# tudelft/event_flow

Hardware: AMD Instinct MI355X
Metric: event-windows/sec (train step, 128x128x15k ev) (higher is better)
Workload: dtype f32

## Files before the change

event_flow_amd/_lib.py:

```python

import ctypes
import os

import torch

_HERE = os.path.dirname(os.path.abspath(__file__))
LIB_PATH = os.environ.get("EVF_LIB") or os.path.join(_HERE, "libevflow_hip.so")

P = ctypes.c_void_p
I = ctypes.c_int
F = ctypes.c_float
L = ctypes.c_int64

SIGNATURES = {
    "evf_version": [],
    "evf_device_count": [],
    "evf_events_to_image": [P, P, P, I, I, I, I, P, P],
    "evf_encode_events": [P, I, I, I, I, I, I, P, P, P, P, P],
    "evf_encode_window": [P, I, I, I, I, I, I, I, I, P, P, P],
    "evf_iwe_splat": [P, P, P, P, P, P, I, I, I, I, I, F, F, F, I, I, P, P],
    "evf_get_interpolation": [P, P, I, I, I, I, F, F, I, P, P, P],
    "evf_interpolate": [P, P, P, I, I, I, I, I, P, P],
    "evf_cm_smooth_blocks": [I, I, I, I],
    "evf_norm_nonzero": [P, ctypes.c_int64, P, P, P],
# ... 62 lines not shown
    "evf_head_dgrad_win_fits": [I, I, I, I, I, I, I, I, I],
    "evf_head_dgrad_win_select": [I, I],
    "evf_head_bwd_dgrad_win": [P, P, P, P, P, P, P, P, P, I, I, I, I, I, I, F, P, P, P, P, I, P],
    "evf_sum_rows": [P, I, I, I, P, P],
    "evf_add_segments": [P, P, P, P, I, I, P],
    "evf_pack_conv_weights_b3_multi": [P, P, P, I, P],
    "evf_reduce_slabs_multi": [P, P, I, I, I, P],
    "evf_lif_bwd_wgrad": [P, P, P, P, P, P, P, P, P, I, I, I, I, I, F, P, P, P, P, P, P, P, I, P],
    "evf_lif_bwd_wgrad2": [P, P, P, P, P, P, P, P, P, P, I, I, I, I, I, F, P, P, P, P, P, P, P, I, P],
    "evf_lif_bwd_wgrad_top": [P, P, P, P, P, P, P, P, P, P, P, P, P, I, I, I, I, I, F, P, P, P, P, P, P, I, P],
    "evf_debug_poison_lds": [ctypes.c_uint32, P],
    "evf_memset": [P, I, ctypes.c_size_t, P],
    "evf_plif_bwd_wgrad2": [P, P, P, P, P, P, P, P, P, P, I, I, I, I, I, F, P, P, P, P, P, P, P, I, P, P, P, P, P, P, P, P, P, P],
    "evf_conv_dgrad_b3_multi": [I, P, P, P, P, P, I, I, I, P],
    "evf_conv_dgrad_b3_multi_fits": [I, I, I],
    "evf_lif_bwd_wgrad_window": [I, P, P, P, P, P, P, P, P, P, P, P, P, P, P, P, I, I, I, F, P, P, P, P, I, P],
    "evf_plif_bwd_wgrad_window_top": [I, P, P, P, P, P, P, P, P, P, P, P, P, P, P, P, P, P, P, P, I, I, I, F, P, P, P, P, P, P, P, I, P],
    "evf_plif_bwd_wgrad_window": [I, P, P, P, P, P, P, P, P, P, P, P, P, P, P, I, I, I, F, P, P, P, P, P, P, P, I, P],
    "evf_plif_bwd_wgrad_top": [P, P, P, P, P, P, P, P, P, P, P, P, P, I, I, I, I, I, F, P, P, P, P, P, P, I,
                               P, P, P, P, P, P, P, P, P, P],
    "evf_pack_conv_weight_b3t": [P, I, I, P, P],
    "evf_conv_dgrad_b3": [P, P, P, I, I, I, I, P, P, P],
    "evf_conv_dgrad_b3_f32": [P, P, P, I, I, I, I, P, P, P],
    "evf_conv_dgrad_select": [I],
    "evf_dgrad_diag_select": [I],
    "evf_bwd_diag_select": [I],
    "evf_bwd_leak_defer": [],
    "evf_fwd_diag_select": [I],
    "evf_conv_dgrad_b3_f32_pair": [P, P, P, I, P, P, I, I, I, P, P, P],
    "evf_conv_dgrad_b3_pair": [P, P, P, I, P, P, I, I, I, P, P, P],
# ... 295 lines not shown
```

event_flow_amd/csrc/evf_bwd_fused.hip:

```cpp
#include <stdio.h>

#include "evf_common.h"
#include "evf_split.h"
#include <stdlib.h>
#include <mutex>

typedef float f32x16 __attribute__((ext_vector_type(16)));
typedef __bf16 bf16x8 __attribute__((ext_vector_type(8)));

#define C32 32
#define FB_CW 64
#define FB_UNITS 8
#define FB_UNITS_MAX 64
#define FB_THREADS 512
#define FB_NW (FB_CW / 32 + 2)
#define FB_R0 32768

#define FB_LD_SKIP 16
#define FB_LD_COLLECT 32
#define FB_LD_MIN_LEAK (-11.0f)

__device__ __forceinline__ int fb_row(int r, int lane) { return (r & 3) + 8 * (r >> 2) + 4 * (lane >> 5); }
__device__ __forceinline__ float fb_sigmoid(float x) { return 1.0f / (1.0f + expf(-x)); }
__device__ __forceinline__ uint32_t fb_bf16(float f) {
// ... 226 lines not shown
        dlam = vp[c] * (1.0f - z) - cur;
      } else {
        gp[c] = gv * lam[c];
        cur = (vo[c] - vp[c] * lam[c] + z * th[c]) * inv_oml[c];
        dlam = vp[c] - cur;
        if (ok) st[c] -= gv * z;
      }
      if (ok) {
        sl[c] += gv * dlam;
        st[c] -= gsp;
      }
    }
    if (ok) {
#ifdef FB_NT_STORES
      if (g_cur) g_cur[pix0 * 8 + tid] = make_float4(gc[0], gc[1], gc[2], gc[3]);
      evf_store_nt(g_v_prev + pix0 * 8 + tid, make_float4(gp[0], gp[1], gp[2], gp[3]));
#else
      if (g_cur) g_cur[pix0 * 8 + tid] = make_float4(gc[0], gc[1], gc[2], gc[3]);
      g_v_prev[pix0 * 8 + tid] = make_float4(gp[0], gp[1], gp[2], gp[3]);
#endif
    }
    uint32_t tp[3][2];
    const int base = ((p >> 3) * C32) * 8 + (p & 7);
#pragma unroll
    for (int e = 0; e < 2; ++e) {
      evf_split3_pair(ok ? gc[2 * e] : 0.f, ok ? gc[2 * e + 1] : 0.f, tp[0][e], tp[1][e], tp[2][e]);
#pragma unroll
      for (int t3 = 0; t3 < 3; ++t3) {
        const int o = t3 * FB_CW * C32 + base + (4 * cg + 2 * e) * 8;
        sb[o] = (unsigned short)tp[t3][e];
        sb[o + 8] = (unsigned short)(tp[t3][e] >> 16);
      }
    }
    if (ok && g_split) {
// ... 503 lines not shown
          if (LD && ld_collect) sl[c] += (vo[c] * inv_oml[c]) * (gvo[c] * inv_lam[c]);
          st[c] -= gsp;
        }
        }
      }
      const long eo = pix0 * 8 + ETHR * h + et;
      if (WIN) {
        gvc = make_float4(gp[0], gp[1], gp[2], gp[3]);
        voc = vp4;
        if (ok) {
          if (w_gcur) w_gcur[eo] = make_float4(gc[0], gc[1], gc[2], gc[3]);
          if (ks == T - 1 && g_v_prev) g_v_prev[eo] = gvc;
        }
      } else if (ok) {
        if (g_cur) g_cur[eo] = make_float4(gc[0], gc[1], gc[2], gc[3]);
        g_v_prev[eo] = make_float4(gp[0], gp[1], gp[2], gp[3]);
      }
      if (PLIF) {
        const float4 gk4 = WIN ? (ks > 0 ? gkc : z4) : (has_gk ? sp.gk : z4), pp4 = (WIN ? w_pp : has_pp) ? sp.pp : z4;
        const float gk[4] = {gk4.x, gk4.y, gk4.z, gk4.w}, pp[4] = {pp4.x, pp4.y, pp4.z, pp4.w};
        const float Pv = sp.P;
        float gq[4], gPp = 0.f, gzx[4];
#pragma unroll
        for (int c = 0; c < 4; ++c) {
          const float po = pov[c];
          const float gx = xl ? gsv[c] : gc[c];
          const float g = gk[c] - apt[c] * gx;
          gq[c] = g * lpt[c];
          if constexpr (SOFT) gq[c] -= gzs[c] * apt[c];
          gzx[c] = g * (1.0f - lpt[c]);
          gPp += gzx[c];
// ... 903 lines not shown
  evf_bwd_defer_tab[c].active = false;
  evf_ctx_drop(c);
  return rc;
}

static int fb_launch(const float* g_z_out, const float* g_z_out2, const FbTop* topp, const float* g_v_out, const float* v_out, const float* v_prev,
                     const uint32_t* z_prev, const uint32_t* xT, const uint32_t* zT_prev, const float* leak,
                     const float* thresh, int B, int H, int W, int hard_reset, int surrogate, float act_width,
                     float* g_cur, void* g_split, float* g_v_prev, float* g_leak, float* g_thresh, float* slab_ff,
                     float* slab_rec, int accumulate, void* stream, const FbPlif* plp_ = nullptr) {
  if (plp_ && !((hard_reset != 0 || plp_->xl != 0) && surrogate == EVF_ARCTAN)) return EVF_ENOTSUP;
  FbPlif pl_arg = plp_ ? *plp_ : FbPlif{};
  pl_arg.soft = (plp_ && hard_reset == 0) ? 1 : 0;
  const FbPlif* plp = plp_ ? &pl_arg : nullptr;
  if (plp && plp->xl == 2 && topp) return EVF_ENOTSUP;
  if (!v_out || !xT || !leak || !thresh || (!g_cur && !g_split) || !g_v_prev || !g_leak || !g_thresh || !slab_ff || B <= 0 || H <= 0 ||
      W <= 0 || ((zT_prev != nullptr) != (slab_rec != nullptr)) || (topp && (g_z_out || zT_prev)) || (topp && g_z_out2))
    return EVF_EINVAL;
  const int row_ld = accumulate >> 8;
  const int ldf = (fb_leak_defer_env() && !plp) ? (accumulate & (FB_LD_SKIP | FB_LD_COLLECT)) : 0;
  accumulate = (accumulate & 1) | ldf;
  const long nunits = fb_units(B, H, W);
  const int nchunk = (W + FB_CW - 1) / FB_CW;
  const int nrows_all = fb_rows(nunits);
  dim3 grid(fb_blocks_per_cell(nunits, 1)), block(FB_THREADS);
  hipStream_t st = EVF_STREAM(stream);
  const FbTop top = topp ? *topp : FbTop{nullptr, nullptr, nullptr, nullptr, nullptr, nullptr};
  static bool attr[12] = {false};
  const bool fast = (hard_reset != 0 || plp != nullptr) && surrogate == EVF_ARCTAN;
  const int bctx = evf_ctx_find(stream);
  const EvfBwdDefer evf_bwd_defer = bctx >= 0 ? evf_bwd_defer_tab[bctx] : EvfBwdDefer{false, 0, false};
// ... 251 lines not shown
```

event_flow_amd/csrc/evf_common.h:

```cpp
#pragma once
#include <hip/hip_runtime.h>
#include <stdint.h>

#include "../../include/evflow.h"

#define EVF_STREAM(s) ((hipStream_t)(s))

static inline int evf_status() {
  hipError_t e = hipGetLastError();
  return e == hipSuccess ? EVF_OK : -(1000 + (int)e);
}
static inline int evf_hip(hipError_t e) { return e == hipSuccess ? EVF_OK : -(1000 + (int)e); }

#define EVF_KSZ_OK(k) ((k) == 1 || (k) == 3 || (k) == 5 || (k) == 7)

static inline int evf_cdiv(long a, long b) { return (int)((a + b - 1) / b); }

template <auto KERNEL>
static inline void evf_dynamic_lds_once(size_t bytes) {
  static const hipError_t once = hipFuncSetAttribute((const void*)KERNEL, hipFuncAttributeMaxDynamicSharedMemorySize, (int)bytes);
  (void)once;
}

static __global__ void k_evf_fill(uint32_t* __restrict__ dst, uint32_t word, size_t nwords, unsigned char* __restrict__ tail, int ntail,
// ... 132 lines not shown
      s += (raw ? in : (dy == 1 && dx == 1)) ? v : 0.f;
    }
  return raw ? (s / 9.0f) / 32.0f : s;
}

int evf_dgrad_ws_launch(const float* g_cur, const void* wT_b3, float* g_x, int accumulate, int B, int H, int W, const float* g_P,
                        const uint32_t* x_bits, const void* wT2_b3, float* g_x2, int max_blocks, void* stream);

#define EVF_DG_MAX_PROD 16
struct EvfDgProd {
  const void* g;
  const void* wt;
  float* gx;
  const float* gP;
  const uint32_t* xb;
};
struct EvfDgProds {
  EvfDgProd p[EVF_DG_MAX_PROD];
};
int evf_dgrad_diag_ws_launch(const EvfDgProds& P, int nprod, int B, int H, int W, void* stream);
int evf_dgrad_diag_dma_launch(const EvfDgProds& P, int nprod, int B, int H, int W, void* stream);
bool evf_dgrad_diag_fits(int split, int B, int H, int W);

#define EVF_HDW_MAX_P 16
struct EvfHdwArgs {
  const void* g[EVF_HDW_MAX_P];
  const float* v_prev[EVF_HDW_MAX_P];
  const uint32_t* z_prev[EVF_HDW_MAX_P];
  const float* x_in[EVF_HDW_MAX_P];
  const void* wt;
// ... 37 lines not shown
```

event_flow_amd/csrc/evf_dgrad_b3.hip:

```cpp
#include "evf_common.h"
#include "evf_dgrad_mma.h"
#include "evf_split.h"
#include <stdlib.h>

typedef float f32x16 __attribute__((ext_vector_type(16)));
typedef __bf16 bf16x8 __attribute__((ext_vector_type(8)));

#define C32 32
#define DG_ROWS 8
#define NFRAG 54

__device__ __forceinline__ int dg_row(int r, int lane) { return (r & 3) + 8 * (r >> 2) + 4 * (lane >> 5); }
__device__ __forceinline__ uint32_t dg_bf16(float f) {
  const uint32_t u = __float_as_uint(f);
  return (u + 0x7FFFu + ((u >> 16) & 1u)) >> 16;
}

__global__ void k_pack_conv_weight_b3t(const float* __restrict__ w, uint4* __restrict__ dst) {
  const int idx = blockIdx.x * blockDim.x + threadIdx.x;
  if (idx >= 18 * 64) return;
  const int lane = idx & 63, tm = idx >> 6, m = tm & 1, tau = tm >> 1;
  const int j = lane & 31, kg = lane >> 5;
  uint32_t t[3][8];
  for (int e = 0; e < 8; ++e) {
// ... 211 lines not shown
                                                                    const float* __restrict__ gPb,
                                                                    const uint32_t* __restrict__ xbits,
                                                                    const uint4* __restrict__ wt2,
                                                                    float* __restrict__ gx2) {
  dg_body<F32IN, ACC, PLIF, PAIR>(blockIdx.z, gridDim.z, gs, plane_stride, wt, gx, accumulate, B, H, W, gPb, xbits, wt2, gx2);
}

#define DG_MAX_JOBS 8
struct DgJob {
  const uint4* gs;
  const uint4* wt;
  float* gx;
  const uint4* wt2;
  float* gx2;
  int split;
};
struct DgJobs {
  DgJob j[DG_MAX_JOBS];
};
__global__ __launch_bounds__(DG_ROWS * 64) void k_dgrad_diag(DgJobs jobs, int B, int H, int W, int zb) {
  const int jb = blockIdx.z / zb, zz = blockIdx.z - jb * zb;
  const DgJob& J = jobs.j[jb];
  if (J.wt2)
    dg_body<true, false, false, true>(zz, zb, J.gs, 0, J.wt, J.gx, 0, B, H, W, nullptr, nullptr, J.wt2, J.gx2);
  else
    dg_body<true, false, false, false>(zz, zb, J.gs, 0, J.wt, J.gx, 0, B, H, W, nullptr, nullptr, nullptr, nullptr);
}

struct DgDefer {
  int B, H, W, split;
// ... 31 lines not shown
int evf_dg_defer_pending(int ctx, int d) { return dg_tab[ctx].n[d]; }
int evf_dg_defer_launch(int ctx, int d, void* stream) {
  DgDefer& dg_defer = dg_tab[ctx];
  const int n = dg_defer.n[d];
  if (!n) return EVF_OK;
  static const bool env_ws = []() {
    const char* e = getenv("EVF_DGRAD_DIAG");
    return !(e && e[0] == 'l');
  }();
  if (dg_defer.split || (dg_diag_select < 0 ? env_ws : dg_diag_select == 1)) {
    EvfDgProds P;
    int np = 0;
    for (int k = 0; k < n; ++k) {
      const DgJob& J = dg_defer.job[d][k];
      P.p[np++] = EvfDgProd{J.gs, J.wt, J.gx};
      if (J.wt2) P.p[np++] = EvfDgProd{J.gs, J.wt2, J.gx2};
    }
    for (int k = np; k < EVF_DG_MAX_PROD; ++k) P.p[k] = P.p[0];
    evf_prof_mark(2, 0, stream);
    const int rc = dg_defer.split ? evf_dgrad_diag_dma_launch(P, np, dg_defer.B, dg_defer.H, dg_defer.W, stream)
                                  : evf_dgrad_diag_ws_launch(P, np, dg_defer.B, dg_defer.H, dg_defer.W, stream);
    evf_prof_mark(2, 1, stream);
    dg_defer.n[d] = 0;
    return rc;
  }
  const size_t lds = dg_lds_bytes();
  static bool attr_set = false;
  if (!attr_set) {
    (void)hipFuncSetAttribute((const void*)k_dgrad_diag, hipFuncAttributeMaxDynamicSharedMemorySize, (int)lds);
    attr_set = true;
  }
// ... 11 lines not shown
static int dg_select = -1;
extern "C" int evf_conv_dgrad_select(int which) {
  if (which < -1 || which > 1) return EVF_EINVAL;
  dg_select = which;
  return EVF_OK;
}

static int dg_launch(const void* g, int f32in, const void* wT_b3, float* g_x, int accumulate, int B, int H, int W,
                     const float* g_P, const uint32_t* x_bits, const void* wT2_b3, float* g_x2, void* stream) {
  if (!g || !wT_b3 || !g_x || B <= 0 || H <= 0 || W <= 0 || ((g_P != nullptr) != (x_bits != nullptr)) ||
      ((wT2_b3 != nullptr) != (g_x2 != nullptr)))
    return EVF_EINVAL;
  const int bctx = evf_ctx_find(stream);
  const EvfBwdDefer evf_bwd_defer = bctx >= 0 ? evf_bwd_defer_tab[bctx] : EvfBwdDefer{false, 0, false};
  DgDefer& dg_defer = dg_tab[bctx < 0 ? 0 : bctx];
  if (evf_bwd_defer.active) {
    const bool any = evf_dg_defer_count(bctx) != 0;
    const int split = f32in ? 0 : 1;
    const bool same = !any || (dg_defer.B == B && dg_defer.H == H && dg_defer.W == W && dg_defer.split == split);
    if (!accumulate && !g_P && same && dg_defer.n[evf_bwd_defer.slot] < DG_MAX_JOBS && evf_dgrad_diag_fits(split, B, H, W)) {
      dg_defer.B = B, dg_defer.H = H, dg_defer.W = W, dg_defer.split = split;
      dg_defer.job[evf_bwd_defer.slot][dg_defer.n[evf_bwd_defer.slot]++] =
          DgJob{(const uint4*)g, (const uint4*)wT_b3, g_x, (const uint4*)wT2_b3, g_x2, split};
      return EVF_OK;
    }
    const int rc = evf_bwd_defer_flush_now(bctx, stream);
    if (rc) return rc;
  }
  if (f32in) {
    int mode = dg_select;
    if (mode < 0) {
      static const int env_mode = []() {
        const char* e = getenv("EVF_DGRAD");
        return !e ? -1 : (e[0] == 'l' ? 0 : (e[0] == 'w' ? 1 : -1));
      }();
      mode = env_mode;
    }
    if (mode < 0) mode = ((long)B * evf_cdiv(H, 4) * evf_cdiv(W, 32) >= 6L * 256) ? 1 : 0;
    if (mode == 1)
      return evf_dgrad_ws_launch((const float*)g, wT_b3, g_x, accumulate, B, H, W, g_P, x_bits, wT2_b3, g_x2, 0, stream);
// ... 72 lines not shown
```

event_flow_amd/csrc/evf_dgrad_diag.hip:

```cpp
#include "evf_common.h"
#include "evf_dgrad_mma.h"
#include "evf_split.h"
#include <stdlib.h>
#include <type_traits>

typedef float f32x16 __attribute__((ext_vector_type(16)));
typedef __attribute__((address_space(3))) void wd_lds_void;
typedef __attribute__((address_space(1))) const void wd_glb_void;

#define C32 32
#define WD_ROWS 4
#define WD_HW 34
#define WD_HP ((WD_ROWS + 2) * WD_HW)
#define WD_NFRAG 54
#define WD_PLANE (WD_HP * 4)
#define WD_BUF (3 * WD_PLANE)
#define WD_ITEMS (WD_HP * 4)
#define WD_NIT ((WD_ITEMS + 255) / 256)
#define WD_SP 36
#define WD_LDS ((size_t)(WD_NFRAG * 64 + 2 * WD_BUF) * sizeof(uint4) + (size_t)WD_ROWS * 32 * WD_SP * 4)

#ifndef WD_PF
#define WD_PF 2
#endif
// ... 177 lines not shown
      __syncthreads();
    }
  }
  WD_STAMP();
}

#define WM_UPP 13
#define WM_PLANE (WM_UPP * 64)
#define WM_BUF (3 * WM_PLANE)
#define WM_NU (3 * WM_UPP)
#define WM_NJ ((WM_NU + 3) / 4)
#define WM_LDS ((size_t)(WD_NFRAG * 64 + 2 * WM_BUF) * sizeof(uint4) + (size_t)4 * 32 * WD_SP * 4)
#ifndef WM_STAGE
#define WM_STAGE 0
#endif
#ifndef WM_PIPE
#define WM_PIPE 1
#endif

__device__ uint4 wm_zero_page[16];

#ifdef WD_STAMPS
__device__ unsigned long long wm_stamps[16 * 4 * 128];
extern "C" int evf_debug_wm_stamps(void* dst) { return evf_hip(hipMemcpyFromSymbol(dst, HIP_SYMBOL(wm_stamps), sizeof(wm_stamps))); }
#define WM_STAMP()                                                                              \
  do {                                                                                          \
    if (blockIdx.x < 16 && lane == 0 && (wv & 3) == 0 && nst < 128)                             \
      wm_stamps[(blockIdx.x * 4 + (wv >> 2)) * 128 + nst++] = __builtin_readcyclecounter();     \
  } while (0)
#else
#define WM_STAMP() do {} while (0)
#endif

struct WmTile {
  int prod, b, y0, x0;
  const char* g;
  float* gx;
  const float* gP;
  const uint32_t* xb;
};

template <bool FULL, bool PLIFT = false>
__global__ __launch_bounds__(512) void k_dgrad_diag_dma(EvfDgProds P, unsigned plane_bytes, int H, int W, int ntx, int nty,
                                                        unsigned ntiles, unsigned total) {
  extern __shared__ __attribute__((aligned(16))) char smem_raw[];
  uint4* s_w = (uint4*)smem_raw;
  uint4* s_a = s_w + WD_NFRAG * 64;
  float* s_stage = (float*)(s_a + 2 * WM_BUF);
  const int tid = threadIdx.x, lane = tid & 63, wv = tid >> 6;
  const int i = lane & 31, kg = lane >> 5;
  int nst = 0;
  (void)nst;
  WM_STAMP();
  const unsigned lo = (unsigned)(((unsigned long long)blockIdx.x * total) / gridDim.x);
  const unsigned hi = (unsigned)(((unsigned long long)(blockIdx.x + 1) * total) / gridDim.x);
  const int nitem = (int)(hi - lo);
  if (nitem <= 0) return;
// ... 8 lines not shown
  auto item_of = [&](int k, WmTile& t) {
    const unsigned id = lo + (unsigned)min(k, nitem - 1);
    unsigned pr, tl, r, tx, b, ty;
    divmod(id, ntiles, rnt, pr, tl);
#ifdef WM_PROBE_COLMAJOR
    divmod(tl, (unsigned)nty, rnty, r, ty);
    divmod(r, (unsigned)ntx, rntx, b, tx);
#else
    divmod(tl, (unsigned)ntx, rntx, r, tx);
    divmod(r, (unsigned)nty, rnty, b, ty);
#endif
    t.prod = __builtin_amdgcn_readfirstlane((int)pr), t.x0 = __builtin_amdgcn_readfirstlane((int)tx * 32);
    t.b = __builtin_amdgcn_readfirstlane((int)b), t.y0 = __builtin_amdgcn_readfirstlane((int)ty * WD_ROWS);
    t.g = (const char*)P.p[t.prod].g, t.gx = P.p[t.prod].gx;
    if (PLIFT) t.gP = P.p[t.prod].gP, t.xb = P.p[t.prod].xb;
  };
  auto load_weights4 = [&](const uint4* src) {
    for (int u = wv - 4; u < WD_NFRAG; u += 4)
      __builtin_amdgcn_global_load_lds((wd_glb_void*)(src + u * 64 + lane), (wd_lds_void*)(s_w + u * 64), 16, 0, 0);
  };
  int p_hr[WM_NJ], p_hc[WM_NJ], p_lds[WM_NJ];
  unsigned p_off[WM_NJ];
#pragma unroll
  for (int j = 0; j < WM_NJ; ++j) {
    const int q = min((wv & 3) + 4 * j, WM_NU - 1), pl = q / WM_UPP, u = q - pl * WM_UPP;
    const int p = 16 * u + (lane >> 2), pc = min(p, WD_HP - 1);
    p_hr[j] = pc / WD_HW, p_hc[j] = pc - p_hr[j] * WD_HW;
    p_off[j] = (unsigned)pl * plane_bytes + (unsigned)(((lane & 3) ^ ((p >> 2) & 3)) * 16);
    p_lds[j] = __builtin_amdgcn_readfirstlane(pl * WM_PLANE + u * 64);
  }
// ... 26 lines not shown
  };
  float4 ev[4];
  auto epi_read = [&](int r) {
    const int p = 8 * r + (lane >> 3), c4 = (lane & 7) * 4;
    ev[r] = *(const float4*)(st + p * WD_SP + c4);
  };
  float gpv[9];
  uint32_t xbv = 0u;
  auto plif_load = [&](int r, const WmTile& t) {
    if (PLIFT && t.gP) {
      const int p = 8 * r + (lane >> 3);
      const int y = min(t.y0 + wv, H - 1), x = min(t.x0 + p, W - 1);
      evf_plif_gp_load(t.gP, 1, t.b, y, x, H, W, gpv);
      xbv = t.xb[((long)t.b * H + y) * W + x];
    }
  };
  auto epi_store = [&](int r, const WmTile& t) {
    const int y = t.y0 + wv;
    const int p = 8 * r + (lane >> 3), c4 = (lane & 7) * 4;
    float* dst = t.gx + ((unsigned)((t.b * H + y) * W + t.x0 + p) * (unsigned)C32 + (unsigned)c4);
    if (PLIFT && t.gP) {
      const float pv = evf_plif_gp_sum(1, min(y, H - 1), min(t.x0 + p, W - 1), H, W, gpv);
      const uint32_t xq = xbv >> c4;
      ev[r].x += (xq & 1u) ? pv : 0.f, ev[r].y += (xq & 2u) ? pv : 0.f, ev[r].z += (xq & 4u) ? pv : 0.f, ev[r].w += (xq & 8u) ? pv : 0.f;
    }
    if (FULL || (y < H && t.x0 + p < W)) evf_store_nt(dst, ev[r]);
  };
  WmTile cur, nxt, prv;
  int wprod;
  const bool loader = wv >= 4;
// ... 49 lines not shown
#endif
      WM_STAMP();
      __syncthreads();
      if (k + 1 < nitem && nxt.prod != wprod) {
        wprod = nxt.prod;
        load_weights4((const uint4*)P.p[wprod].wt);
        asm volatile("s_waitcnt vmcnt(0)" ::: "memory");
        __syncthreads();
      }
    }
  } else {
    f32x16 acc_prev = {0};
    auto run_item = [&](int k, auto epi_tag) {
      constexpr bool EPI = decltype(epi_tag)::value;
      WM_STAMP();
      auto side = [&](int slot) {
        if (slot == 70) item_of(k + 1, nxt);
        if (EPI) {
          if (slot == 1) epi_write(acc_prev);
#pragma unroll
          for (int r = 0; r < 4; ++r) {
            if (slot == 13 + r) epi_read(r);
            if (PLIFT && slot == 32 + 12 * r) plif_load(r, prv);
            if (slot == 40 + 12 * r) epi_store(r, prv);
          }
        }
      };
      const f32x16 acc = dg_matrix_phase3<WD_DPPX != 0>(s_w, s_a + (k & 1) * WM_BUF, WM_PLANE, wv * WD_HW + i, lane, side);
      WM_STAMP();
      if (!WM_PIPE) {
        epi_write(acc);
        __builtin_amdgcn_wave_barrier();
#pragma unroll
        for (int r = 0; r < 4; ++r) epi_read(r);
#pragma unroll
        for (int r = 0; r < 4; ++r) {
          plif_load(r, cur);
          epi_store(r, cur);
        }
        __builtin_amdgcn_wave_barrier();
      }
      acc_prev = acc;
      prv = cur;
      WM_STAMP();
      __syncthreads();
      if (k + 1 < nitem && nxt.prod != wprod) {
        wprod = nxt.prod;
        __syncthreads();
      }
      cur = nxt;
    };
    WM_STAMP();
    __syncthreads();
    prv = cur;
    run_item(0, std::false_type{});
    for (int k = 1; k < nitem; ++k) run_item(k, std::integral_constant<bool, WM_PIPE != 0>{});
    if (WM_PIPE) {
      epi_write(acc_prev);
      __builtin_amdgcn_wave_barrier();
#pragma unroll
      for (int r = 0; r < 4; ++r) epi_read(r);
#pragma unroll
      for (int r = 0; r < 4; ++r) {
        plif_load(r, prv);
        epi_store(r, prv);
      }
    }
  }
  WM_STAMP();
}

extern int evf_dgrad_ring_select;
#define WR_ROWS 12
#define WR_PITCH 36
#define WR_UPP 27
#define WR_PLANE (WR_UPP * 64)
// ... 238 lines not shown
  if (!attr) {
    (void)hipFuncSetAttribute((const void*)k_dgrad_diag_dma<true>, hipFuncAttributeMaxDynamicSharedMemorySize, (int)WM_LDS);
    (void)hipFuncSetAttribute((const void*)k_dgrad_diag_dma<false>, hipFuncAttributeMaxDynamicSharedMemorySize, (int)WM_LDS);
    attr = true;
  }
  const int nblk = (int)(total < ncu ? total : ncu);
  bool plift = false;
  for (int k = 0; k < nprod; ++k) {
    plift = plift || P.p[k].gP != nullptr;
    if (P.p[k].gP && !P.p[k].xb) return EVF_EINVAL;
  }
  static const bool ring_env = []() {
    const char* e = getenv("EVF_DGRAD_RING");
    return e && e[0] == '1';
  }();
  const bool ring = !plift && (evf_dgrad_ring_select < 0 ? ring_env : evf_dgrad_ring_select == 1);
  if (ring) {
    static bool rattr = false;
    if (!rattr) {
      (void)hipFuncSetAttribute((const void*)k_dgrad_diag_ring<true>, hipFuncAttributeMaxDynamicSharedMemorySize, (int)WR_LDS);
      (void)hipFuncSetAttribute((const void*)k_dgrad_diag_ring<false>, hipFuncAttributeMaxDynamicSharedMemorySize, (int)WR_LDS);
      rattr = true;
    }
    if (H % WD_ROWS == 0 && W % 32 == 0)
      hipLaunchKernelGGL(k_dgrad_diag_ring<true>, dim3(nblk), dim3(512), WR_LDS, EVF_STREAM(stream), P, (unsigned)plane_bytes, H, W,
                         ntx, nty, (unsigned)ntiles, (unsigned)total);
    else
      hipLaunchKernelGGL(k_dgrad_diag_ring<false>, dim3(nblk), dim3(512), WR_LDS, EVF_STREAM(stream), P, (unsigned)plane_bytes, H, W,
                         ntx, nty, (unsigned)ntiles, (unsigned)total);
    return evf_status();
// ... 15 lines not shown
  }
  if (H % WD_ROWS == 0 && W % 32 == 0)
    hipLaunchKernelGGL(k_dgrad_diag_dma<true>, dim3(nblk), dim3(512), WM_LDS, EVF_STREAM(stream), P, (unsigned)plane_bytes, H, W, ntx,
                       nty, (unsigned)ntiles, (unsigned)total);
  else
    hipLaunchKernelGGL(k_dgrad_diag_dma<false>, dim3(nblk), dim3(512), WM_LDS, EVF_STREAM(stream), P, (unsigned)plane_bytes, H, W, ntx,
                       nty, (unsigned)ntiles, (unsigned)total);
  return evf_status();
}

int evf_dgrad_diag_ws_launch(const EvfDgProds& P, int nprod, int B, int H, int W, void* stream) {
  if (nprod <= 0 || nprod > EVF_DG_MAX_PROD || B <= 0 || H <= 0 || W <= 0) return EVF_EINVAL;
  const int ntx = evf_cdiv(W, 32), nty = evf_cdiv(H, WD_ROWS);
  const long ntiles = (long)ntx * nty * B, total = ntiles * nprod;
  if (total >= (1L << 22)) return EVF_EINVAL;
  static int ncu = 0;
  if (!ncu) {
    int dev = 0;
    hipDeviceProp_t pr;
    if (hipGetDevice(&dev) == hipSuccess && hipGetDeviceProperties(&pr, dev) == hipSuccess) ncu = pr.multiProcessorCount;
    if (ncu <= 0) ncu = 256;
  }
  static bool attr = false;
  if (!attr) {
    (void)hipFuncSetAttribute((const void*)k_dgrad_diag_ws, hipFuncAttributeMaxDynamicSharedMemorySize, (int)WD_LDS);
    attr = true;
  }
  const int nblk = (int)(total < ncu ? total : ncu);
  hipLaunchKernelGGL(k_dgrad_diag_ws, dim3(nblk), dim3(512), WD_LDS, EVF_STREAM(stream), P, H, W, ntx, nty, (unsigned)ntiles,
                     (unsigned)total);
  return evf_status();
}

extern "C" int evf_conv_dgrad_b3_multi(int nprod, const void* const* g_split, const void* const* wT_b3, void* const* g_x,
                                       const void* const* g_P_raw, const void* const* x_bits, int B, int H, int W, void* stream) {
  if (nprod <= 0 || nprod > EVF_DG_MAX_PROD || !g_split || !wT_b3 || !g_x) return EVF_EINVAL;
  if (!evf_dgrad_diag_fits(1, B, H, W)) return EVF_ENOTSUP;
  EvfDgProds P;
  for (int k = 0; k < EVF_DG_MAX_PROD; ++k) {
    const int q = k < nprod ? k : 0;
    if (!g_split[q] || !wT_b3[q] || !g_x[q]) return EVF_EINVAL;
    const float* gp = g_P_raw ? (const float*)g_P_raw[q] : nullptr;
    const uint32_t* xb = x_bits ? (const uint32_t*)x_bits[q] : nullptr;
    if ((gp != nullptr) != (xb != nullptr)) return EVF_EINVAL;
    P.p[k] = EvfDgProd{g_split[q], wT_b3[q], (float*)g_x[q], gp, xb};
  }
  evf_prof_mark(9, 0, stream);
  const int rc = evf_dgrad_diag_dma_launch(P, nprod, B, H, W, stream);
  evf_prof_mark(9, 1, stream);
  return rc;
}
extern "C" int evf_conv_dgrad_b3_multi_fits(int B, int H, int W) { return evf_dgrad_diag_fits(1, B, H, W) ? 1 : 0; }
```

event_flow_amd/models/engine.py:

```python

import ctypes
import os

import torch

from .. import _lib
from . import hip_ops
from .spiking_util import SURROGATE_ID

C = 32


def _i32(shape, dev):
    return torch.empty(shape, dtype=torch.int32, device=dev)


def _f32(shape, dev):
    return torch.empty(shape, dtype=torch.float32, device=dev)


F32_DGRAD = os.environ.get("EVF_F32_DGRAD", "1") != "0"
SPLIT_DGRAD = os.environ.get("EVF_DGRAD_SPLIT", "1") != "0"
HEAD_WIN = os.environ.get("EVF_HEAD_WIN", "1") != "0"
PRED_FUSED = os.environ.get("EVF_PRED_FUSED", "1") != "0"
TOP_FUSED = os.environ.get("EVF_TOP_FUSED", "1") != "0"
PAIR_DGRAD = os.environ.get("EVF_PAIR_DGRAD", "1") != "0"
PLIF_BOX_IN_DGRAD = os.environ.get("EVF_PLIF_BOX", "dgrad") != "kernel"
PLIF_TRACE_FUSED = os.environ.get("EVF_PLIF_TRACE_FUSED", "1") != "0"
PLIF_LAYER_MAJOR = os.environ.get("EVF_PLIF_LAYER_MAJOR", "1") != "0"
PLIF_LM_DGRAD = os.environ.get("EVF_PLIF_LM_DGRAD", "ws")
LIF_BWD_TOP = os.environ.get("EVF_LIF_BWD_TOP", "1") != "0"
FWD_LAYER_MAJOR = os.environ.get("EVF_FWD_LM", "auto")
FWD_LM_MIN_QUADS = int(os.environ.get("EVF_FWD_LM_MIN_QUADS", "1024"))
FWD_LM_PASSES = 16
FUSED_TAIL = os.environ.get("EVF_FUSED_TAIL", "1") != "0"
PARAM_ROWS = os.environ.get("EVF_PARAM_ROWS", "1") != "0"


class _Window:

    def __init__(self, eng, B, H, W, dev):
        n = len(eng.cells)
        self.shape = (B, H, W)
        self.dev = dev
        self.gv = [None] * n
        self.gz = [None] * n
# ... 1 lines not shown
        self.g_cur = None
        self.g_split = None
        self.gpt = [None] * n
        self.gpt_has = [False] * n
        self.ld_owed = [None] * n
        self.gP = None
        self.small, self.small_persistent = eng._take_small(dev)
        self.rows = eng._take_rows(B, H, W, dev)
        n_ = len(eng.cells)
        self.gzr, self.gzr_has = [None] * n_, [False] * n_
        self.gcl = [None] * n_
        self.gsl = [None] * n_
        self.gz0 = []
        self.gsl1 = []
        self.gs0 = None
        self.bwd_k = 0
        self.lm = []
        self.slab_init = {}
        self.head_det_rows = 0
        self.det = False
        self.token = eng._token(dev)
        self.n_passes = 0
        self.flow_buf = _f32((eng._flow_cap, B, 2, H, W), dev)

    def buf(self, lst, l):
        if lst[l] is None:
            B, H, W = self.shape
            lst[l] = _f32((B, H, W, C), self.dev)
        return lst[l]

# ... 514 lines not shown
            top = i == n - 1
            kf = (i, "ff")
            _lib.call("evf_lif_bwd_wgrad_window", T, None if top else arr([gz(i, s_) for s_ in range(T)]),
                      arr([tp["flow"] for tp in tapes]) if top else None, arr(gflows) if top else None,
                      _lib.ptr(self._flat["pred.w"]) if top else None, arr([l_[4] for l_ in lay]) if top else None,
                      rowp("pred.w") if top else None, rowp("pred.b") if top else None, arr([l_[3] for l_ in lay]),
                      arr([l_[1] for l_ in lay]), arr([l_[2] for l_ in lay]), arr([l_[5] for l_ in lay]), None, arr(gsp),
                      _lib.ptr(self._flat[f"{i}.leak"]), _lib.ptr(self._flat[f"{i}.thresh"]), B, H, W, self._act_width(i), None,
                      rowp(f"{i}.leak"), rowp(f"{i}.thresh"), _lib.ptr(self._slab(kf, nsl, dev)),
                      (1 if win.slab_init.get(kf) else 0) | (row_ld << 8))
            win.slab_init[kf] = True
            _lib.call("evf_conv_dgrad_b3_multi", T, arr(gsp), arr([self._packed[(i, "ff", "b3t")]] * T),
                      arr([gz(i - 1, s_) for s_ in range(T)]), None, None, B, H, W)
        for s_ in range(T):
            win.gz[last_rec], win.gz_has[last_rec] = gz(last_rec, s_), True
            self._backward_pass(win, tapes[s_], None, firsts[s_])
            win.bwd_k += 1

    def _lm_replay(self, win):
        stash, win.lm = win.lm, []
        for tape, g_flow, is_first in stash:
            self._backward_pass(win, tape, g_flow, is_first)
            win.bwd_k += 1

    def _lm_buf(self, key, shape, dev, dtype=torch.float32):
        d = self.__dict__.setdefault("_lm_bufs", {})
        k = (key, tuple(shape), str(dev))
        if k not in d:
            d[k] = torch.empty(shape, dtype=dtype, device=dev)
        return d[k]

    def _backward_window_lm(self, win):
# ... 181 lines not shown
            use_rec = c.recurrent and z_prev is not None
            split = bdefer and SPLIT_DGRAD and i > 0
            if split and hdw_i:
                while len(win.gsl1) <= win.bwd_k:
                    win.gsl1.append(self._lm_buf(("gsl1", len(win.gsl1)), (3, B, H, W, C), dev, torch.bfloat16))
                g_cur_i, g_split_i = None, win.gsl1[win.bwd_k]
            elif split:
                if win.gsl[i] is None:
                    win.gsl[i] = torch.empty((3, B, H, W, C), dtype=torch.bfloat16, device=dev)
                g_cur_i, g_split_i = None, win.gsl[i]
            else:
                g_cur_i = win.buf(win.gcl, i) if bdefer else win.g_cur
                g_split_i = win.g_split
            if bdefer:
                self._bdefer_slot(win, 2 * (n - 1 - i))
            gv_out = win.buf(win.gv, i)
            leak_g, thr_g = self._small(win, f"{i}.leak"), self._small(win, f"{i}.thresh")
            (leak_r, row_ld), (thr_r, _) = self._rowed(win, f"{i}.leak"), self._rowed(win, f"{i}.thresh")
            trace_fused = (plif and PLIF_TRACE_FUSED and PLIF_BOX_IN_DGRAD and i > 0 and self.precision == "bf16x3"
                           and (c.hard_reset or self._xsoft) and c.activation == "arctanspike")
            if (self._xl or self._al) and ((i > 0 and not trace_fused) or (i == 0 and tape["x_in"].shape[1] != 2)):
                raise _lib.EvflowError("fused XLIF / ALIF cells need the trace backward inside the fused backward kernels (EVF_PLIF_TRACE_FUSED, "
                                       "EVF_PLIF_BOX=dgrad, a two-channel input); EVF_XLIF_FUSED=0 serves the network on the general path")
            if trace_fused:
                if win.gP is None:
                    win.gP = _f32((B, H, W), dev)
                    win.gP_raw = _f32((B, H, W), dev)
                gpt_out = win.buf(win.gpt, i)
                gzx_buf = win.buf(win.gzr, i) if self._al else None
                trace_args = (_lib.ptr(gpt_out if win.gpt_has[i] else None), _lib.ptr(pt_prev), _lib.ptr(P_sav),
                              _lib.ptr(self._flat[f"{i}.leak_pt"]), _lib.ptr(self._flat[f"{i}.add_pt"]), _lib.ptr(gpt_out),
# ... 131 lines not shown
                    continue
                if (bdefer or plif_hw) and i == 1 and HEAD_WIN and not win.gz_has[0]:
                    while len(win.gz0) <= win.bwd_k:
                        win.gz0.append(_f32((B, H, W, C), dev))
                    win.gz[0] = win.gz0[win.bwd_k]
                ga = win.buf(win.gz, i - 1)
                acc_a = 1 if win.gz_has[i - 1] else 0
                trace_in = plif and not self._al
                gp_flag = 2 if (trace_in and PLIF_BOX_IN_DGRAD) else 0
                gp_map = (win.gP_raw if PLIF_BOX_IN_DGRAD else win.gP) if trace_in else None
                if self.precision == "bf16x3":
                    dg, gsrc = ("evf_conv_dgrad_b3_f32", g_cur_i) if F32_DGRAD else ("evf_conv_dgrad_b3", win.g_split)
                    if split:
                        dg, gsrc = "evf_conv_dgrad_b3", g_split_i
                    if rec_grad and (F32_DGRAD or split) and PAIR_DGRAD and not self._al:
                        gb = win.buf(win.gzr, i) if not plif else win.buf(win.gz, i)
                        _lib.call("evf_conv_dgrad_b3_pair" if split else "evf_conv_dgrad_b3_f32_pair", _lib.ptr(gsrc),
                                  _lib.ptr(self._packed[(i, "ff", "b3t")]),
                                  _lib.ptr(ga), acc_a | gp_flag, _lib.ptr(self._packed[(i, "rec", "b3t")]), _lib.ptr(gb), B, H, W,
                                  _lib.ptr(gp_map) if trace_in else None, _lib.ptr(in_bits) if trace_in else None)
                        if plif:
                            win.gz_has[i] = True
                        else:
                            win.gzr_has[i] = True
                    else:
                        _lib.call(dg, _lib.ptr(gsrc), _lib.ptr(self._packed[(i, "ff", "b3t")]), _lib.ptr(ga),
                                  acc_a | gp_flag, B, H, W, _lib.ptr(gp_map) if trace_in else None, _lib.ptr(in_bits) if trace_in else None)
                        if rec_grad and self._al:
                            _lib.call(dg, _lib.ptr(gsrc), _lib.ptr(self._packed[(i, "rec", "b3t")]),
                                      _lib.ptr(win.buf(win.gzr, i)), 1, B, H, W, None, None)
                        elif rec_grad:
                            gb = win.buf(win.gz, i)
                            _lib.call(dg, _lib.ptr(gsrc), _lib.ptr(self._packed[(i, "rec", "b3t")]),
                                      _lib.ptr(gb), 0, B, H, W, None, None)
                            win.gz_has[i] = True
                elif rec_grad:
# ... 125 lines not shown
```

include/evflow.h:

```cpp
#ifndef EVFLOW_H
#define EVFLOW_H

#include <stdint.h>

#ifdef __cplusplus
extern "C" {
#endif

#define EVF_OK 0
#define EVF_EINVAL (-22)
#define EVF_ENOTSUP (-95)

int evf_version(void);
int evf_device_count(void);

int evf_events_to_image(const float* xs, const float* ys, const float* vals, int n,
                        int H, int W, int accumulate, float* out, void* stream);

int evf_encode_events(const float* ev, int B, int N, int H, int W, int num_bins, int round_ts,
                      float* cnt, float* mask, float* voxel, float* pol, void* stream);
int evf_encode_window(const float* ev, int B, int P, int N, int H, int W, int num_bins, int round_ts, int want,
                      float* dense, float* pol, void* stream);

int evf_iwe_splat(const float* flow, const float* ev, const int32_t* map_of_event, const int32_t* ts_shift,
// ... 128 lines not shown
                          float* g_cur, void* g_split, float* g_v_prev, float* g_leak, float* g_thresh,
                          float* slab_ff, int accumulate, void* stream);

int evf_pack_conv_weight_b3t(const float* w, int Cout, int Cin, void* dst, void* stream);
int evf_pack_conv_weights_b3_multi(const void* const* w, void* const* dst_b3, void* const* dst_b3t, int count, void* stream);
int evf_conv_dgrad_b3(const void* g_split, const void* wT_b3, float* g_x, int accumulate,
                      int B, int H, int W, const float* g_P, const uint32_t* x_bits, void* stream);
int evf_conv_dgrad_b3_f32(const float* g_cur, const void* wT_b3, float* g_x, int accumulate,
                          int B, int H, int W, const float* g_P, const uint32_t* x_bits, void* stream);
int evf_conv_dgrad_b3_pair(const void* g_split, const void* wT_b3, float* g_x, int accumulate,
                           const void* wT2_b3, float* g_x2, int B, int H, int W,
                           const float* g_P, const uint32_t* x_bits, void* stream);
int evf_conv_dgrad_b3_multi(int nprod, const void* const* g_split, const void* const* wT_b3, void* const* g_x,
                            const void* const* g_P_raw, const void* const* x_bits, int B, int H, int W, void* stream);
int evf_conv_dgrad_b3_multi_fits(int B, int H, int W);
int evf_conv_dgrad_select(int which);
int evf_dgrad_diag_select(int which);
int evf_fwd_diag_select(int which);
int evf_bwd_diag_select(int which);
int evf_bwd_leak_defer(void);
int evf_conv_dgrad_b3_f32_pair(const float* g_cur, const void* wT_b3, float* g_x, int accumulate,
                               const void* wT2_b3, float* g_x2, int B, int H, int W,
                               const float* g_P, const uint32_t* x_bits, void* stream);

int evf_conv_plif_fwd_b3(const uint32_t* x, const void* wb_ff, const void* wb_rec,
                         const float* leak_v, const float* leak_pt, const float* add_pt, const float* thresh,
                         const float* v_prev, const uint32_t* z_prev, const float* pt_prev,
                         int B, int H, int W, int hard_reset,
                         float* v_out, uint32_t* z_out, uint32_t* zT_out, float* pt_out, float* P_out, void* stream);
int evf_conv_plif_fwd_b3_pred(const uint32_t* x, const void* wb_ff, const void* wb_rec,
// ... 285 lines not shown
```

Before: 2664.

## Accumulate recurrent dgrad into next step's gradient and skip dead g_v_prev stores

Adds an accumulate mode to the deferred multi-product dgrad kernel, so the recurrent-weight dgrad can read-add-write directly into the next timestep's gz buffer instead of writing a separate gzr buffer that is summed later. That path is only taken when EVF_DGRAD_SUM=2. With the default setting, the backward LIF kernel now skips writing g_v_prev for the first layer step when that output is provably unused, which saves a full-resolution store. The accumulate path adds an extra global read in the epilogue and restrictions that make it return ENOTSUP on aliasing or PLIF cases.

```diff
diff --git a/event_flow_amd/_lib.py b/event_flow_amd/_lib.py
--- a/event_flow_amd/_lib.py
+++ b/event_flow_amd/_lib.py
@@ -100,6 +100,7 @@
     "evf_plif_bwd_wgrad2": [P, P, P, P, P, P, P, P, P, P, I, I, I, I, I, F, P, P, P, P, P, P, P, I, P, P, P, P, P, P, P, P, P, P],
     "evf_conv_dgrad_b3_multi": [I, P, P, P, P, P, I, I, I, P],
     "evf_conv_dgrad_b3_multi_fits": [I, I, I],
+    "evf_conv_dgrad_b3_multi_acc": [I, P, P, P, P, I, I, I, P],
     "evf_lif_bwd_wgrad_window": [I, P, P, P, P, P, P, P, P, P, P, P, P, P, P, P, I, I, I, F, P, P, P, P, I, P],
     "evf_plif_bwd_wgrad_window_top": [I, P, P, P, P, P, P, P, P, P, P, P, P, P, P, P, P, P, P, P, I, I, I, F, P, P, P, P, P, P, P, I, P],
     "evf_plif_bwd_wgrad_window": [I, P, P, P, P, P, P, P, P, P, P, P, P, P, P, I, I, I, F, P, P, P, P, P, P, P, I, P],
diff --git a/event_flow_amd/csrc/evf_bwd_fused.hip b/event_flow_amd/csrc/evf_bwd_fused.hip
--- a/event_flow_amd/csrc/evf_bwd_fused.hip
+++ b/event_flow_amd/csrc/evf_bwd_fused.hip
@@ -264,10 +264,10 @@
     if (ok) {
 #ifdef FB_NT_STORES
       if (g_cur) g_cur[pix0 * 8 + tid] = make_float4(gc[0], gc[1], gc[2], gc[3]);
-      evf_store_nt(g_v_prev + pix0 * 8 + tid, make_float4(gp[0], gp[1], gp[2], gp[3]));
+      if (g_v_prev) evf_store_nt(g_v_prev + pix0 * 8 + tid, make_float4(gp[0], gp[1], gp[2], gp[3]));
 #else
       if (g_cur) g_cur[pix0 * 8 + tid] = make_float4(gc[0], gc[1], gc[2], gc[3]);
-      g_v_prev[pix0 * 8 + tid] = make_float4(gp[0], gp[1], gp[2], gp[3]);
+      if (g_v_prev) g_v_prev[pix0 * 8 + tid] = make_float4(gp[0], gp[1], gp[2], gp[3]);
 #endif
     }
     uint32_t tp[3][2];
@@ -801,7 +801,7 @@
         }
       } else if (ok) {
         if (g_cur) g_cur[eo] = make_float4(gc[0], gc[1], gc[2], gc[3]);
-        g_v_prev[eo] = make_float4(gp[0], gp[1], gp[2], gp[3]);
+        if (PLIF || g_v_prev) g_v_prev[eo] = make_float4(gp[0], gp[1], gp[2], gp[3]);
       }
       if (PLIF) {
         const float4 gk4 = WIN ? (ks > 0 ? gkc : z4) : (has_gk ? sp.gk : z4), pp4 = (WIN ? w_pp : has_pp) ? sp.pp : z4;
@@ -1735,7 +1735,7 @@
   pl_arg.soft = (plp_ && hard_reset == 0) ? 1 : 0;
   const FbPlif* plp = plp_ ? &pl_arg : nullptr;
   if (plp && plp->xl == 2 && topp) return EVF_ENOTSUP;
-  if (!v_out || !xT || !leak || !thresh || (!g_cur && !g_split) || !g_v_prev || !g_leak || !g_thresh || !slab_ff || B <= 0 || H <= 0 ||
+  if (!v_out || !xT || !leak || !thresh || (!g_cur && !g_split) || (!g_v_prev && plp) || !g_leak || !g_thresh || !slab_ff || B <= 0 || H <= 0 ||
       W <= 0 || ((zT_prev != nullptr) != (slab_rec != nullptr)) || (topp && (g_z_out || zT_prev)) || (topp && g_z_out2))
     return EVF_EINVAL;
   const int row_ld = accumulate >> 8;
diff --git a/event_flow_amd/csrc/evf_common.h b/event_flow_amd/csrc/evf_common.h
--- a/event_flow_amd/csrc/evf_common.h
+++ b/event_flow_amd/csrc/evf_common.h
@@ -170,6 +170,7 @@
   float* gx;
   const float* gP;
   const uint32_t* xb;
+  int acc;
 };
 struct EvfDgProds {
   EvfDgProd p[EVF_DG_MAX_PROD];
diff --git a/event_flow_amd/csrc/evf_dgrad_b3.hip b/event_flow_amd/csrc/evf_dgrad_b3.hip
--- a/event_flow_amd/csrc/evf_dgrad_b3.hip
+++ b/event_flow_amd/csrc/evf_dgrad_b3.hip
@@ -249,6 +249,7 @@
   const uint4* wt2;
   float* gx2;
   int split;
+  int acc2;
 };
 struct DgJobs {
   DgJob j[DG_MAX_JOBS];
@@ -310,7 +311,7 @@
     for (int k = 0; k < n; ++k) {
       const DgJob& J = dg_defer.job[d][k];
       P.p[np++] = EvfDgProd{J.gs, J.wt, J.gx};
-      if (J.wt2) P.p[np++] = EvfDgProd{J.gs, J.wt2, J.gx2};
+      if (J.wt2) P.p[np++] = EvfDgProd{J.gs, J.wt2, J.gx2, nullptr, nullptr, J.acc2};
     }
     for (int k = np; k < EVF_DG_MAX_PROD; ++k) P.p[k] = P.p[0];
     evf_prof_mark(2, 0, stream);
@@ -352,6 +353,9 @@
   const int bctx = evf_ctx_find(stream);
   const EvfBwdDefer evf_bwd_defer = bctx >= 0 ? evf_bwd_defer_tab[bctx] : EvfBwdDefer{false, 0, false};
   DgDefer& dg_defer = dg_tab[bctx < 0 ? 0 : bctx];
+  const int acc2 = (accumulate & 4) ? 1 : 0;
+  accumulate &= ~4;
+  if (acc2 && (f32in || !wT2_b3 || !evf_bwd_defer.active)) return EVF_ENOTSUP;
   if (evf_bwd_defer.active) {
     const bool any = evf_dg_defer_count(bctx) != 0;
     const int split = f32in ? 0 : 1;
@@ -359,9 +363,10 @@
     if (!accumulate && !g_P && same && dg_defer.n[evf_bwd_defer.slot] < DG_MAX_JOBS && evf_dgrad_diag_fits(split, B, H, W)) {
       dg_defer.B = B, dg_defer.H = H, dg_defer.W = W, dg_defer.split = split;
       dg_defer.job[evf_bwd_defer.slot][dg_defer.n[evf_bwd_defer.slot]++] =
-          DgJob{(const uint4*)g, (const uint4*)wT_b3, g_x, (const uint4*)wT2_b3, g_x2, split};
+          DgJob{(const uint4*)g, (const uint4*)wT_b3, g_x, (const uint4*)wT2_b3, g_x2, split, acc2};
       return EVF_OK;
     }
+    if (acc2) return EVF_ENOTSUP;
     const int rc = evf_bwd_defer_flush_now(bctx, stream);
     if (rc) return rc;
   }
diff --git a/event_flow_amd/csrc/evf_dgrad_diag.hip b/event_flow_amd/csrc/evf_dgrad_diag.hip
--- a/event_flow_amd/csrc/evf_dgrad_diag.hip
+++ b/event_flow_amd/csrc/evf_dgrad_diag.hip
@@ -215,6 +215,9 @@
 #ifndef WM_STAGE
 #define WM_STAGE 0
 #endif
+#ifndef WM_ACC_READ
+#define WM_ACC_READ 34
+#endif
 #ifndef WM_PIPE
 #define WM_PIPE 1
 #endif
@@ -239,9 +242,10 @@
   float* gx;
   const float* gP;
   const uint32_t* xb;
+  int acc;
 };
 
-template <bool FULL, bool PLIFT = false>
+template <bool FULL, bool PLIFT = false, bool ACC = false>
 __global__ __launch_bounds__(512) void k_dgrad_diag_dma(EvfDgProds P, unsigned plane_bytes, int H, int W, int ntx, int nty,
                                                         unsigned ntiles, unsigned total) {
   extern __shared__ __attribute__((aligned(16))) char smem_raw[];
@@ -280,6 +284,7 @@
     t.b = __builtin_amdgcn_readfirstlane((int)b), t.y0 = __builtin_amdgcn_readfirstlane((int)ty * WD_ROWS);
     t.g = (const char*)P.p[t.prod].g, t.gx = P.p[t.prod].gx;
     if (PLIFT) t.gP = P.p[t.prod].gP, t.xb = P.p[t.prod].xb;
+    if (ACC) t.acc = P.p[t.prod].acc;
   };
   auto load_weights4 = [&](const uint4* src) {
     for (int u = wv - 4; u < WD_NFRAG; u += 4)
@@ -336,6 +341,17 @@
       evf_plif_gp_load(t.gP, 1, t.b, y, x, H, W, gpv);
       xbv = t.xb[((long)t.b * H + y) * W + x];
     }
+  };
+  auto acc_load = [&](int r, const WmTile& t, float4* ov) {
+    if (ACC) {
+      const int p = 8 * r + (lane >> 3), c4 = (lane & 7) * 4;
+      const int y = FULL ? t.y0 + wv : min(t.y0 + wv, H - 1), x = FULL ? t.x0 + p : min(t.x0 + p, W - 1);
+      const float* src = t.gx + ((unsigned)((t.b * H + y) * W + x) * (unsigned)C32 + (unsigned)c4);
+      ov[r] = *(const float4*)(t.acc ? (const char*)src : zero_page);
+    }
+  };
+  auto acc_add = [&](int r, const WmTile& t, const float4* ov) {
+    if (ACC && t.acc) ev[r].x = ov[r].x + ev[r].x, ev[r].y = ov[r].y + ev[r].y, ev[r].z = ov[r].z + ev[r].z, ev[r].w = ov[r].w + ev[r].w;
   };
   auto epi_store = [&](int r, const WmTile& t) {
     const int y = t.y0 + wv;
@@ -415,13 +431,16 @@
     auto run_item = [&](int k, auto epi_tag) {
       constexpr bool EPI = decltype(epi_tag)::value;
       WM_STAMP();
+      float4 ov[4];
       auto side = [&](int slot) {
         if (slot == 70) item_of(k + 1, nxt);
         if (EPI) {
           if (slot == 1) epi_write(acc_prev);
 #pragma unroll
           for (int r = 0; r < 4; ++r) {
-            if (slot == 13 + r) epi_read(r);
+            if (ACC && slot == 3 + r) acc_load(r, prv, ov);
+            if (slot == (ACC ? WM_ACC_READ + r : 13 + r)) epi_read(r);
+            if (ACC && slot == WM_ACC_READ + 2 + r) acc_add(r, prv, ov);
             if (PLIFT && slot == 32 + 12 * r) plif_load(r, prv);
             if (slot == 40 + 12 * r) epi_store(r, prv);
           }
@@ -435,6 +454,10 @@
 #pragma unroll
         for (int r = 0; r < 4; ++r) epi_read(r);
 #pragma unroll
+        for (int r = 0; r < 4; ++r) acc_load(r, cur, ov);
+#pragma unroll
+        for (int r = 0; r < 4; ++r) acc_add(r, cur, ov);
+#pragma unroll
         for (int r = 0; r < 4; ++r) {
           plif_load(r, cur);
           epi_store(r, cur);
@@ -457,10 +480,15 @@
     run_item(0, std::false_type{});
     for (int k = 1; k < nitem; ++k) run_item(k, std::integral_constant<bool, WM_PIPE != 0>{});
     if (WM_PIPE) {
+      float4 ov[4];
       epi_write(acc_prev);
       __builtin_amdgcn_wave_barrier();
 #pragma unroll
+      for (int r = 0; r < 4; ++r) acc_load(r, prv, ov);
+#pragma unroll
       for (int r = 0; r < 4; ++r) epi_read(r);
+#pragma unroll
+      for (int r = 0; r < 4; ++r) acc_add(r, prv, ov);
 #pragma unroll
       for (int r = 0; r < 4; ++r) {
         plif_load(r, prv);
@@ -729,6 +757,29 @@
     const char* e = getenv("EVF_DGRAD_RING");
     return e && e[0] == '1';
   }();
+  bool accp = false;
+  for (int k = 0; k < nprod; ++k) {
+    if (!P.p[k].acc) continue;
+    accp = true;
+    for (int j = 0; j < nprod; ++j)
+      if (j != k && P.p[j].gx == P.p[k].gx) return EVF_ENOTSUP;
+  }
+  if (accp) {
+    if (plift) return EVF_ENOTSUP;
+    static bool aattr = false;
+    if (!aattr) {
+      (void)hipFuncSetAttribute((const void*)k_dgrad_diag_dma<true, false, true>, hipFuncAttributeMaxDynamicSharedMemorySize, (int)WM_LDS);
+      (void)hipFuncSetAttribute((const void*)k_dgrad_diag_dma<false, false, true>, hipFuncAttributeMaxDynamicSharedMemorySize, (int)WM_LDS);
+      aattr = true;
+    }
+    if (H % WD_ROWS == 0 && W % 32 == 0)
+      hipLaunchKernelGGL((k_dgrad_diag_dma<true, false, true>), dim3(nblk), dim3(512), WM_LDS, EVF_STREAM(stream), P, (unsigned)plane_bytes, H,
+                         W, ntx, nty, (unsigned)ntiles, (unsigned)total);
+    else
+      hipLaunchKernelGGL((k_dgrad_diag_dma<false, false, true>), dim3(nblk), dim3(512), WM_LDS, EVF_STREAM(stream), P, (unsigned)plane_bytes, H,
+                         W, ntx, nty, (unsigned)ntiles, (unsigned)total);
+    return evf_status();
+  }
   const bool ring = !plift && (evf_dgrad_ring_select < 0 ? ring_env : evf_dgrad_ring_select == 1);
   if (ring) {
     static bool rattr = false;
@@ -774,6 +825,8 @@
   const int ntx = evf_cdiv(W, 32), nty = evf_cdiv(H, WD_ROWS);
   const long ntiles = (long)ntx * nty * B, total = ntiles * nprod;
   if (total >= (1L << 22)) return EVF_EINVAL;
+  for (int k = 0; k < nprod; ++k)
+    if (P.p[k].acc) return EVF_ENOTSUP;
   static int ncu = 0;
   if (!ncu) {
     int dev = 0;
@@ -792,8 +845,8 @@
   return evf_status();
 }
 
-extern "C" int evf_conv_dgrad_b3_multi(int nprod, const void* const* g_split, const void* const* wT_b3, void* const* g_x,
-                                       const void* const* g_P_raw, const void* const* x_bits, int B, int H, int W, void* stream) {
+static int dgrad_b3_multi(int nprod, const void* const* g_split, const void* const* wT_b3, void* const* g_x,
+                          const void* const* g_P_raw, const void* const* x_bits, const int* acc, int B, int H, int W, void* stream) {
   if (nprod <= 0 || nprod > EVF_DG_MAX_PROD || !g_split || !wT_b3 || !g_x) return EVF_EINVAL;
   if (!evf_dgrad_diag_fits(1, B, H, W)) return EVF_ENOTSUP;
   EvfDgProds P;
@@ -803,11 +856,20 @@
     const float* gp = g_P_raw ? (const float*)g_P_raw[q] : nullptr;
     const uint32_t* xb = x_bits ? (const uint32_t*)x_bits[q] : nullptr;
     if ((gp != nullptr) != (xb != nullptr)) return EVF_EINVAL;
-    P.p[k] = EvfDgProd{g_split[q], wT_b3[q], (float*)g_x[q], gp, xb};
+    P.p[k] = EvfDgProd{g_split[q], wT_b3[q], (float*)g_x[q], gp, xb, (acc && k < nprod && acc[k]) ? 1 : 0};
+    if (P.p[k].acc && gp) return EVF_ENOTSUP;
   }
   evf_prof_mark(9, 0, stream);
   const int rc = evf_dgrad_diag_dma_launch(P, nprod, B, H, W, stream);
   evf_prof_mark(9, 1, stream);
   return rc;
 }
+extern "C" int evf_conv_dgrad_b3_multi(int nprod, const void* const* g_split, const void* const* wT_b3, void* const* g_x,
+                                       const void* const* g_P_raw, const void* const* x_bits, int B, int H, int W, void* stream) {
+  return dgrad_b3_multi(nprod, g_split, wT_b3, g_x, g_P_raw, x_bits, nullptr, B, H, W, stream);
+}
+extern "C" int evf_conv_dgrad_b3_multi_acc(int nprod, const void* const* g_split, const void* const* wT_b3, void* const* g_x,
+                                           const int* acc, int B, int H, int W, void* stream) {
+  return dgrad_b3_multi(nprod, g_split, wT_b3, g_x, nullptr, nullptr, acc, B, H, W, stream);
+}
 extern "C" int evf_conv_dgrad_b3_multi_fits(int B, int H, int W) { return evf_dgrad_diag_fits(1, B, H, W) ? 1 : 0; }
diff --git a/event_flow_amd/models/engine.py b/event_flow_amd/models/engine.py
--- a/event_flow_amd/models/engine.py
+++ b/event_flow_amd/models/engine.py
@@ -30,6 +30,8 @@
 PLIF_LAYER_MAJOR = os.environ.get("EVF_PLIF_LAYER_MAJOR", "1") != "0"
 PLIF_LM_DGRAD = os.environ.get("EVF_PLIF_LM_DGRAD", "ws")
 LIF_BWD_TOP = os.environ.get("EVF_LIF_BWD_TOP", "1") != "0"
+DGRAD_SUM = os.environ.get("EVF_DGRAD_SUM", "1") != "0"
+DGRAD_SUM_G2 = os.environ.get("EVF_DGRAD_SUM", "1") == "2"
 FWD_LAYER_MAJOR = os.environ.get("EVF_FWD_LM", "auto")
 FWD_LM_MIN_QUADS = int(os.environ.get("EVF_FWD_LM_MIN_QUADS", "1024"))
 FWD_LM_PASSES = 16
@@ -61,6 +63,7 @@
         self.gz0 = []
         self.gsl1 = []
         self.gs0 = None
+        self.gz_sum = None
         self.bwd_k = 0
         self.lm = []
         self.slab_init = {}
@@ -605,8 +608,10 @@
                       arr([gz(i - 1, s_) for s_ in range(T)]), None, None, B, H, W)
         for s_ in range(T):
             win.gz[last_rec], win.gz_has[last_rec] = gz(last_rec, s_), True
+            win.gz_sum = (last_rec, gz(last_rec, s_ + 1)) if (DGRAD_SUM_G2 and s_ + 1 < T) else None
             self._backward_pass(win, tapes[s_], None, firsts[s_])
             win.bwd_k += 1
+        win.gz_sum = None
 
     def _lm_replay(self, win):
         stash, win.lm = win.lm, []
@@ -818,7 +823,8 @@
                 g_split_i = win.g_split
             if bdefer:
                 self._bdefer_slot(win, 2 * (n - 1 - i))
-            gv_out = win.buf(win.gv, i)
+            gv_dead = (DGRAD_SUM and is_first and i > 0 and self.kind == "lif" and self.precision == "bf16x3" and not self._plif)
+            gv_out = None if gv_dead else win.buf(win.gv, i)
             leak_g, thr_g = self._small(win, f"{i}.leak"), self._small(win, f"{i}.thresh")
             (leak_r, row_ld), (thr_r, _) = self._rowed(win, f"{i}.leak"), self._rowed(win, f"{i}.thresh")
             trace_fused = (plif and PLIF_TRACE_FUSED and PLIF_BOX_IN_DGRAD and i > 0 and self.precision == "bf16x3"
@@ -980,12 +986,19 @@
                     if split:
                         dg, gsrc = "evf_conv_dgrad_b3", g_split_i
                     if rec_grad and (F32_DGRAD or split) and PAIR_DGRAD and not self._al:
-                        gb = win.buf(win.gzr, i) if not plif else win.buf(win.gz, i)
+                        sum_dst = win.gz_sum[1] if (DGRAD_SUM_G2 and split and not plif and win.gz_sum is not None and win.gz_sum[0] == i) else None
+                        if sum_dst is not None:
+                            gb = sum_dst
+                        else:
+                            gb = win.buf(win.gzr, i) if not plif else win.buf(win.gz, i)
                         _lib.call("evf_conv_dgrad_b3_pair" if split else "evf_conv_dgrad_b3_f32_pair", _lib.ptr(gsrc),
                                   _lib.ptr(self._packed[(i, "ff", "b3t")]),
-                                  _lib.ptr(ga), acc_a | gp_flag, _lib.ptr(self._packed[(i, "rec", "b3t")]), _lib.ptr(gb), B, H, W,
+                                  _lib.ptr(ga), acc_a | gp_flag | (4 if sum_dst is not None else 0), _lib.ptr(self._packed[(i, "rec", "b3t")]),
+                                  _lib.ptr(gb), B, H, W,
                                   _lib.ptr(gp_map) if trace_in else None, _lib.ptr(in_bits) if trace_in else None)
-                        if plif:
+                        if sum_dst is not None:
+                            pass
+                        elif plif:
                             win.gz_has[i] = True
                         else:
                             win.gzr_has[i] = True
diff --git a/include/evflow.h b/include/evflow.h
--- a/include/evflow.h
+++ b/include/evflow.h
@@ -166,6 +166,8 @@
 int evf_conv_dgrad_b3_multi(int nprod, const void* const* g_split, const void* const* wT_b3, void* const* g_x,
                             const void* const* g_P_raw, const void* const* x_bits, int B, int H, int W, void* stream);
 int evf_conv_dgrad_b3_multi_fits(int B, int H, int W);
+int evf_conv_dgrad_b3_multi_acc(int nprod, const void* const* g_split, const void* const* wT_b3, void* const* g_x,
+                                const int* acc, int B, int H, int W, void* stream);
 int evf_conv_dgrad_select(int which);
 int evf_dgrad_diag_select(int which);
 int evf_fwd_diag_select(int which);
```

Result: slower. 2626 (-1.4%).
